# UCLA-VAST/soda-compiler

Hardware: AMD Instinct MI355X
Metric: gcell_updates_per_s (higher is better)
Workload: dtype f32; 1 GPU; jacobi2d.soda float32 16384x16384, iterate 1000; app=jacobi2d, valid_cell_updates=236970022000, nominal_cell_updates=268435456000, depth_schedule=41x24+1x16, depth_split=measured (soda_hip_plan_tune), stream_chunk_choice=calibrated (confirmed by measurement), device=gfx950:sramecc+:xnack-

## Files before the change

### soda-compiler_amd/csrc/schedule.cpp

```cpp
#include "schedule.h"

#include <algorithm>
#include <cmath>
#include <cstdarg>
#include <cstdio>
#include <cstdlib>
#include <cstring>

thread_local std::string g_last_error;

int fail(int code, const char* fmt, ...) {
  char buf[1024];
  va_list ap;
  va_start(ap, fmt);
  vsnprintf(buf, sizeof buf, fmt, ap);
  va_end(ap);
  g_last_error = buf;
  return code;
}

const char* tuning_env(const char* name) {
  const char* on = getenv("SODA_HIP_TUNING");
  return (on && on[0] == '1') ? getenv(name) : nullptr;
}
// ... 416 lines not shown
  if (desc.xcd_tiles && dim == 3) return place_super_tiles(plan, k, out);
  return 0;
}

int check_box_inside(const Planner* plan, const soda_hip_args& a,
                     const int32_t* reach_lo, const int32_t* reach_hi,
                     bool signed_window = false) {
  for (int d = 0; d < plan->prog.dim; ++d) {
    if (a.box_hi[d] <= a.box_lo[d]) continue;
    const int64_t first = signed_window ? a.box_lo[d] + reach_lo[d] : a.box_lo[d] - reach_lo[d];
    if (first < 0 || a.box_hi[d] + reach_hi[d] > a.dims[d])
      return fail(SODA_HIP_ERR_OUT_OF_BOUNDS,
                  "launch would read [%lld, %lld) of dimension %d, extent %lld",
                  (long long)first,
                  (long long)(a.box_hi[d] + reach_hi[d]), d, (long long)a.dims[d]);
  }
  return 0;
}

std::vector<int> eligible_fused(const Planner* plan, const int64_t* dims) {
  const soda_hip_program& p = plan->prog;
  std::vector<int> fused;
  for (size_t k = 0; k < plan->kernels.size(); ++k) {
    const soda_hip_kernel& kd = plan->kernels[k];
    if (kd.kind != SODA_HIP_KERNEL_FUSED ||
        (plan->max_depth > 0 && kd.depth > plan->max_depth))
      continue;
    if (kd.min_extent[0] > 0 &&
        (dims[0] < kd.min_extent[0] || (p.dim > 1 && dims[1] < kd.min_extent[1]) ||
         (p.dim > 2 && dims[0] * dims[1] >= (int64_t(1) << 30) - 16)))
      continue;
    fused.push_back((int)k);
  }
  std::sort(fused.begin(), fused.end(), [&](int a, int b) {
    return plan->kernels[a].depth > plan->kernels[b].depth;
  });
  return fused;
}

bool plans_fused(const Planner* plan, const std::vector<int>& fused, const int64_t* dims,
                 int iterate) {
  if (fused.empty() || plan->kernels[fused.back()].depth != 1) return false;
  if (plan->max_depth < 0) return false;
  if (plan->max_depth == 0 && !plan->tuning &&
      (takes_output_extras(plan, plan->kernels[fused.back()]) || plan->prog.dim == 1)) {
    return plan->tuned_split.find(split_key(plan, dims, iterate)) != plan->tuned_split.end();
  }
  return true;
}

soda_hip_args box_of_level(Planner* plan, Growth* g, const int64_t* dims, const int32_t* vlo,
                           const int32_t* vhi, int level, int32_t* mlo, int32_t* mhi) {
  const soda_hip_program& p = plan->prog;
  soda_hip_args a;
  memset(&a, 0, sizeof a);
  hull_margins(plan, g, level, mlo, mhi);
  for (int d = 0; d < SODA_HIP_MAX_DIMS; ++d) {
    a.dims[d] = d < p.dim ? dims[d] : 1;
    a.box_lo[d] = d < p.dim ? vlo[d] + mlo[d] : 0;
    a.box_hi[d] = d < p.dim ? dims[d] - vhi[d] - mhi[d] : 1;
  }
  return a;
}

int split_iterate(Planner* plan, Growth* g, const std::vector<int>& fused, const int64_t* dims,
                  int iterate, const int32_t* vlo, const int32_t* vhi, std::vector<int>* seq) {
  std::vector<int> usable;
// ... 104 lines not shown
                "carry the boxes of %d", desc.name, p.n_outputs, max_extra_outputs(dim));
  const std::vector<Box>& boxes = g->boxes[level - 1];
  for (int j = 0; j < p.n_outputs; ++j) {
    const Box& o = boxes[p.output_tensor[j]];
    int64_t ex[6];
    soda_hip_args own = *a;
    for (int d = 0; d < dim; ++d) {
      ex[d] = mlo[d] + o.lo[d];
      ex[dim + d] = mhi[d] - o.hi[d];
      if (ex[d] < 0 || ex[d] > kMaxExtra || ex[dim + d] < 0 || ex[dim + d] > kMaxExtra)
        return fail(SODA_HIP_ERR_INTERNAL, "kernel %s: output %d is %lld / %lld cells "
                    "wider than the launch's box in dimension %d (limit %d)", desc.name,
                    j, (long long)ex[d], (long long)ex[dim + d], d, kMaxExtra);
      own.box_lo[d] -= ex[d];
      own.box_hi[d] += ex[dim + d];
    }
    const int32_t none[SODA_HIP_MAX_DIMS] = {0, 0, 0, 0};
    int rc = check_box_inside(plan, own, none, none);
    if (rc) return rc;
    uint64_t word = 0;
    for (int i = 0; i < 2 * dim; ++i) word |= (uint64_t)ex[i] << (8 * i);
    if (dim == 1) a->param[1 + j / 4] |= (int64_t)(word << (16 * (j % 4)));
    else if (dim == 2) a->param[1 + j / 2] |= (int64_t)(word << (32 * (j % 2)));
    else a->param[1 + j] = (int64_t)word;
  }
  return 0;
}

int fused_list(Planner* plan, Growth* g, const std::vector<int>& fused, const std::vector<int>& seq,
               const int64_t* dims, const int32_t* vlo, const int32_t* vhi,
               std::vector<Launch>* list, int* max_depth_used, ScratchNeeds* needs) {
  const int m = (int)seq.size();
  int done = 0;
  std::vector<Buffer> src = sweep_inputs(plan);
  for (int i = 0; i < m; ++i) {
    const soda_hip_kernel& desc = plan->kernels[seq[i]];
    Buffer tensor[SODA_HIP_MAX_TENSORS];
    route(plan, i, m, &src, tensor, needs);
    int32_t mlo[SODA_HIP_MAX_DIMS], mhi[SODA_HIP_MAX_DIMS];
    int32_t plo[SODA_HIP_MAX_DIMS], phi[SODA_HIP_MAX_DIMS];
    hull_margins(plan, g, done, plo, phi);
    soda_hip_args a = box_of_level(plan, g, dims, vlo, vhi, done + desc.depth, mlo, mhi);
    int32_t reach_lo[SODA_HIP_MAX_DIMS], reach_hi[SODA_HIP_MAX_DIMS];
    for (int d = 0; d < SODA_HIP_MAX_DIMS; ++d) {
      reach_lo[d] = mlo[d] - plo[d];
      reach_hi[d] = mhi[d] - phi[d];
    }
    int rc = check_box_inside(plan, a, reach_lo, reach_hi);
    if (rc) return rc;
    if (takes_output_extras(plan, desc)) {
      rc = pack_output_extras(plan, g, desc, done + desc.depth, mlo, mhi, &a);
      if (rc) return rc;
    }
    Launch l;
    bool empty;
    rc = make_launch(plan, seq[i], a, &l, &empty);
    if (rc) return rc;
    if (!empty && l.est_us > 0) {
      const char* prefer = tuning_env("SODA_HIP_PREFER");
      auto preferred = [&](int k) {
        if (!prefer) return false;
        const size_t n = strlen(plan->kernels[k].name), m = strlen(prefer);
        return n >= m && strcmp(plan->kernels[k].name + n - m, prefer) == 0;
      };
      for (int k : fused) {
        if (k == seq[i] || plan->kernels[k].depth != desc.depth) continue;
        Launch other;
        bool other_empty;
        if (make_launch(plan, k, a, &other, &other_empty) == 0 && !other_empty &&
            other.est_us > 0 &&
            (preferred(k) || (other.est_us < l.est_us && !preferred(l.kernel))))
          l = other;
      }
    }
    std::copy(tensor, tensor + SODA_HIP_MAX_TENSORS, l.buffer);
    if (!empty) list->push_back(l);
    *max_depth_used = std::max(*max_depth_used, (int)desc.depth);
    done += desc.depth;
  }
  return 0;
}

int staged_list(Planner* plan, const Growth* g, const int64_t* dims, int iterate, const int32_t* vlo,
                const int32_t* vhi, std::vector<Launch>* list, int* max_depth_used,
                ScratchNeeds* needs) {
  const soda_hip_program& p = plan->prog;
  std::vector<int> stage_kernel(p.n_stages, -1);
  for (size_t k = 0; k < plan->kernels.size(); ++k)
    if (plan->kernels[k].kind == SODA_HIP_KERNEL_STAGE) {
      const int s = plan->kernels[k].stage - p.n_inputs;
      if (s >= 0 && s < p.n_stages) stage_kernel[s] = (int)k;
    }
  for (int s = 0; s < p.n_stages; ++s)
    if (stage_kernel[s] < 0)
      return fail(SODA_HIP_ERR_NO_KERNEL, "blob has no kernel for stage %d", s);
  std::vector<Buffer> src = sweep_inputs(plan);
  for (int it = 0; it < iterate; ++it) {
    Buffer tensor[SODA_HIP_MAX_TENSORS];
    for (int s = 0; s < p.n_stages; ++s) {
      if (is_output_tensor(p, p.n_inputs + s)) continue;
      tensor[p.n_inputs + s].kind = Buffer::LOCAL;
      tensor[p.n_inputs + s].index = (uint8_t)s;
      needs->locals = true;
    }
    route(plan, it, iterate, &src, tensor, needs);
// ... 95 lines not shown
```

### soda-compiler_amd/csrc/schedule.h

```cpp
#ifndef SODA_HIP_SCHEDULE_H_
#define SODA_HIP_SCHEDULE_H_

#include "soda_hip.h"

#include <array>
#include <cstdint>
#include <map>
#include <string>
#include <utility>
#include <vector>

struct Box {
  int32_t lo[SODA_HIP_MAX_DIMS];
  int32_t hi[SODA_HIP_MAX_DIMS];
  bool set;
};

struct Buffer {
  enum Kind : uint8_t {
    NONE,
    INPUT,
    OUTPUT,
    ARRAY_A,
    ARRAY_B,
// ... 16 lines not shown

struct ScratchNeeds {
  bool pingpong = false;
  bool second = false;
  bool locals = false;
};

struct Growth {
  std::vector<Box> start;
  std::vector<std::vector<Box>> boxes;
  std::vector<Box> feed;
};

struct Planner {
  soda_hip_program prog{};
  std::vector<soda_hip_kernel> kernels;
  std::vector<int> resident_blocks;
  std::vector<int> static_lds;
  int cus = 256;
  int64_t lds_per_cu = 160 * 1024;
  int max_depth = 0;
  int chunk_rows_override = 0;
  int chunk_rows_min = 8;
  int wgs_per_cu_cap = 0;
  bool out_final_only = false;
  int bias_depth = 0;
  double bias = 1.0;
  bool tuning = false;
  Growth fresh;
  std::map<std::vector<int32_t>, Growth> resumed;
  mutable std::map<std::array<int64_t, 4>, std::pair<int, int>> xcd_shape;
  std::map<std::array<int64_t, 5>, std::vector<int>> tuned_split;
  std::map<std::array<int64_t, 5>, std::array<int, 2>> tuned_stream;
};

#pragma GCC visibility push(hidden)

extern thread_local std::string g_last_error;
int fail(int code, const char* fmt, ...) __attribute__((format(printf, 2, 3)));

const char* tuning_env(const char* name);

int n_tensors(const soda_hip_program& p);
bool is_output_tensor(const soda_hip_program& p, int t);

void output_margins(Planner* plan, int iterations, int32_t* lo, int32_t* hi);
void field_margins(Planner* plan, int iterations, int32_t (*lo)[SODA_HIP_MAX_DIMS],
                   int32_t (*hi)[SODA_HIP_MAX_DIMS]);

std::array<int64_t, 5> split_key(const Planner* plan, const int64_t* dims, int iterate);
std::array<int64_t, 5> stream_key(const Planner* plan, int k, const soda_hip_args& args);

double footprint_of(const Planner* plan, const soda_hip_args& args);
const double kBeyondCacheBytes = 288.0 * 1024 * 1024;

int build_schedule(Planner* plan, const int64_t* dims, int iterate, const int32_t* valid_lo,
                   const int32_t* valid_hi, std::vector<Launch>* list, int* max_depth_used,
                   ScratchNeeds* needs);
int build_schedule_fields(Planner* plan, const int64_t* dims, int iterate,
                          const int32_t (*valid_lo)[SODA_HIP_MAX_DIMS],
                          const int32_t (*valid_hi)[SODA_HIP_MAX_DIMS],
                          std::vector<Launch>* list, int* max_depth_used, ScratchNeeds* needs);

#pragma GCC visibility pop

#endif
// ... 1 lines not shown
```

### soda-compiler_amd/csrc/soda_hip.cpp

```cpp
#include "plan.h"

#include <hip/hiprtc.h>

#include <algorithm>
#include <array>
#include <cmath>
#include <cstdio>
#include <cstdlib>
#include <cstring>
#include <map>
#include <string>
#include <vector>

namespace {

int grow_zeroed(void** array, size_t* have, size_t bytes, hipStream_t stream) {
  if (*have >= bytes) return 0;
  if (*array) {
    HIP_TRY(SODA_HIP_ERR_DEVICE_FREE, hipFree(*array));
    *array = nullptr;
    *have = 0;
  }
  HIP_TRY(SODA_HIP_ERR_DEVICE_MALLOC, hipMalloc(array, bytes));
  HIP_TRY(SODA_HIP_ERR_DEVICE_RUN, hipMemsetAsync(*array, 0, bytes, stream));
// ... 495 lines not shown
    int depth = 0;
    ScratchNeeds needs;
    rc = build_schedule(plan, dims, iterate, valid_lo, valid_hi, &list, &depth, &needs);
    std::vector<int> split;
    for (const Launch& l : list)
      if (plan->kernels[l.kernel].kind == SODA_HIP_KERNEL_FUSED)
        split.push_back(plan->kernels[l.kernel].depth);
    int total = 0;
    for (int d : split) total += d;
    if (!rc && total == iterate &&
        std::find(candidates.begin(), candidates.end(), split) == candidates.end())
      candidates.push_back(split);
  }
  plan->bias_depth = 0;
  plan->bias = 1.0;
  plan->tuning = false;
  if (rc) return rc;
  hipEvent_t e0 = nullptr, e1 = nullptr;
  if (hipEventCreate(&e0) != hipSuccess || hipEventCreate(&e1) != hipSuccess)
    return fail(SODA_HIP_ERR_DEVICE_RUN, "hipEventCreate failed");
  auto time_sweep = [&](int runs, float* fastest) -> int {
    int e = 0;
    for (int run = 0; run <= runs && !e; ++run) {
      if (hipEventRecord(e0, s) != hipSuccess) e = fail(SODA_HIP_ERR_DEVICE_RUN, "hipEventRecord failed");
      if (!e) e = soda_hip_sweep(plan, in, out, dims, iterate, valid_lo, valid_hi, stream);
      if (!e && (hipEventRecord(e1, s) != hipSuccess || hipEventSynchronize(e1) != hipSuccess))
        e = fail(SODA_HIP_ERR_DEVICE_SYNC, "timing a tuning sweep failed");
      float ms = 0;
      if (!e) (void)hipEventElapsedTime(&ms, e0, e1);
      if (run == 1 || (run > 1 && ms < *fastest)) *fastest = ms;
    }
    return e;
  };
  if (candidates.size() < 2) {
    rc = tune_streaming(plan, dims, iterate, valid_lo, valid_hi, time_sweep);
    (void)hipEventDestroy(e0);
    (void)hipEventDestroy(e1);
    return rc;
  }
  size_t best = 0;
  float best_ms = 0;
  for (size_t c = 0; c < candidates.size() && !rc; ++c) {
    plan->tuned_split[key] = candidates[c];
    float fastest = 0;
    rc = time_sweep(2, &fastest);
    if (tuning_env("SODA_HIP_DEBUG")) {
      fprintf(stderr, "soda_hip: tune %d iteration(s):", iterate);
      for (int d : candidates[c]) fprintf(stderr, " %d", d);
      fprintf(stderr, "  -> %.1f us\n", fastest * 1000.0);
    }
    if (c == 0 || fastest < best_ms) { best = c; best_ms = fastest; }
  }
  if (rc) plan->tuned_split.erase(key);
  else plan->tuned_split[key] = candidates[best];
  if (!rc) rc = tune_streaming(plan, dims, iterate, valid_lo, valid_hi, time_sweep);
  (void)hipEventDestroy(e0);
  (void)hipEventDestroy(e1);
  return rc;
}

int soda_hip_plan_set_split(soda_hip_plan* plan, const int64_t dims[SODA_HIP_MAX_DIMS],
                            int iterate, const int32_t* depths, int n_depths) {
  if (!plan || !dims) return fail(SODA_HIP_ERR_NULL_ARGUMENT, "NULL argument");
  const std::array<int64_t, 5> key = split_key(plan, dims, iterate);
  if (!depths || n_depths <= 0) {
    plan->tuned_split.erase(key);
    return 0;
  }
  int total = 0;
  for (int i = 0; i < n_depths; ++i) {
    bool known = false;
    for (const soda_hip_kernel& kd : plan->kernels)
      known = known || (kd.kind == SODA_HIP_KERNEL_FUSED && kd.depth == depths[i]);
    if (!known)
      return fail(SODA_HIP_ERR_NO_KERNEL, "no fused kernel of depth %d in the blob",
                  (int)depths[i]);
    total += depths[i];
  }
  if (total != iterate)
    return fail(SODA_HIP_ERR_CONSTRAINT, "the depths add up to %d, not to iterate = %d",
                total, iterate);
  plan->tuned_split[key] = std::vector<int>(depths, depths + n_depths);
  return 0;
}

int soda_hip_plan_set_out_final_only(soda_hip_plan* plan, int on) {
  if (!plan) return fail(SODA_HIP_ERR_NULL_ARGUMENT, "plan is NULL");
// ... 398 lines not shown
```

### soda-compiler_amd/soda_hip/codegen/kernel.py

```python
import collections
import functools
import hashlib
import inspect
import json
import os
import re
import subprocess
import tempfile

from .. import __version__
from . import (kernel_common, kernel_fields1d, kernel_fields2d, kernel_fields3d, kernel_stage,
               kernel_stream1d, kernel_stream2d, kernel_stream2d_wp, kernel_stream3d,
               kernel_stream3d_blk, kernel_stream3d_lds, kernel_stream3d_wp)
from . import spec as specmod
from . import switches

DEFAULT_MAX_DEPTH = 12
WAVE_GROUPS = -1
AUTO_WP_VGPRS = 200
AUTO_WP_GROUPS = 4
AUTO_WP_BUDGET = 200
AUTO_WP_RING = 6
AUTO_WP_SQUEEZE_VGPRS = 152
PACKED_DEEP_DEPTHS = (16, 20, 24)
PACKED_DEEP_DEPTH = PACKED_DEEP_DEPTHS[0]
PACKED_DEEP_WAVES_PER_EU = 3
PACKED_FROM_DEPTH = 12
WAVE_PIPELINE_MIN_DEPTH = 4
ALIGN_FULL_MAX_DEPTH = 2
NT_AUTO_MAX_DEPTH_2D = 2
EXACT_PREFETCH = 6
DEEP_3D_DEPTHS = (4,)
BLOCK_3D_SHALLOW_DEPTHS = (1, 2)
DEEP_3D_FORM = 'both'
BLOCK_3D_OPTIONS = dict(stack=8, prefetch=1, vgpr_budget=300, nt=4, mask_loads=1,
                        wide_stores=2, edge=1)
BLOCK_3D_RING_OPTIONS = dict(stack=8, prefetch=0, ring=2, vgpr_budget=300, nt=4,
                             mask_loads=1, wide_stores=2, lean_fill=1, edge=1)
DEEP_3D_MAX_WEIGHT = 20
PACKED_3D_LIGHT_WEIGHT = 10
ALIGN_FULL_MAX_WEIGHT = 40

FIELDS_DEPTHS = (1, 2, 4, 8)
FIELDS_OPTIONS = ('skip_fill', 'vgpr_budget', 'max_period', 'waves_per_eu')
FIELDS3D_DEPTHS = (1, 2)
FIELDS3D_OPTIONS = ('rows', 'vgpr_budget', 'max_period', 'waves_per_eu')
RECT3D_INPUT_ROWS = 36
STREAM1D_DEPTHS = (1, 2, 4, 8, 12)
STREAM1D_OPTIONS = ('segs',)
FIELDS1D_OPTIONS = STREAM1D_OPTIONS
LDS3D_OPTIONS = ('lds_shape',)

FAR_MAX_PERIOD = 24

SHARED_2D_OPTIONS = ('skip_fill', 'vgpr_budget', 'max_period', 'align', 'waves_per_eu')
WP_ONLY_OPTIONS = ('pairs', 'ring', 'split', 'prio', 'seam_probe')

HIPCC_FLAGS = ['-x', 'hip', '--offload-arch=gfx950', '--cuda-device-only',
               '--no-gpu-bundle-output', '-O3', '-ffp-contract=off',
               '-fno-slp-vectorize', '-fwrapv', '-std=c++17']


_DOUBLE_LITERAL = re.compile(
    r'(?<![\w.])(?:\d+\.\d*|\.\d+|\d+(?=[eE]))(?:[eE][+-]?\d+)?(?![\w.])')


def dpp_combine_is_safe(spec):
  if any(t != 'float' for t in specmod.tensor_c_types(spec).values()):
    return False
  for stage in spec['stages']:
    for text in [stage['expr']] + [l['expr'] for l in stage['lets']]:
      plain = specmod.LOAD_RE.sub('x', text)
      if _DOUBLE_LITERAL.search(plain) or kernel_common.used_functions(
          dict(stages=[dict(expr=text, lets=[])])) or 'static_cast<' in plain:
        return False
  return True


def extra_flags(spec):
  tuning = []
  if spec['dim'] == 2 and \
      kernel_stream2d_wp.packable(specmod.inline_pointwise(spec)):
    tuning = ['-mllvm', '-amdgpu-sched-strategy=max-ilp']
  if dpp_combine_is_safe(spec):
    return tuning
  return ['-mllvm', '-amdgpu-dpp-combine=false'] + tuning


FLAGS_MARK = '// SODA-HIP-FLAGS:'
# ... 116 lines not shown
    valu = waves * entry['depth'] * weight * lane_cells * 2
    cells_in = waves * kernel_stream2d.LANES * lane_cells
    cells_out = entry['tile'][0] * entry['tile'][1]
  entry['step_valu'] = int(valu)
  entry['step_bytes'] = int((n_in * cells_in + n_out * cells_out) * elem)
  measured = calibration().get(calibration_key(entry, spec))
  if measured:
    for field in CALIBRATED_FIELDS:
      entry[field] = int(measured.get(field, 0))
    for field in MEASURED_OVER_DEFAULT:
      if field in measured:
        entry[field] = int(measured[field])
  return entry


def prefixed_options(options, prefix, emit):
  known = inspect.signature(emit).parameters
  out = {}
  for key, value in options.items():
    if key.startswith(prefix):
      if key[len(prefix):] not in known:
        raise TypeError('%s: %s() has no option `%s`' % (key, emit.__module__,
                                                         key[len(prefix):]))
      out[key[len(prefix):]] = value
  return out



FORM_OPTIONS = dict(
    fields2d=lambda k: k in FIELDS_OPTIONS,
    fields3d=lambda k: k in FIELDS3D_OPTIONS,
    fields1d=lambda k: k in FIELDS1D_OPTIONS,
    stream1d=lambda k: k in STREAM1D_OPTIONS,
    stream2d=lambda k: k not in WP_ONLY_OPTIONS + STREAM1D_OPTIONS and k != 'nt',
    stream2d_wp=lambda k: k in SHARED_2D_OPTIONS + WP_ONLY_OPTIONS,
    stream3d=lambda k: not k.startswith(('wp_', 'blk_')) and
    k not in ('deep3d', 'deep3d_from', 'nontemporal') + STREAM1D_OPTIONS + LDS3D_OPTIONS,
    stream3d_lds=lambda k: k in LDS3D_OPTIONS)
PREFIXED_FORMS = dict(stream3d_blk=('blk_', kernel_stream3d_blk.emit),
                      stream3d_wp=('wp_', kernel_stream3d_wp.emit))


def form_options(form, options):
  if form in PREFIXED_FORMS:
    return prefixed_options(options, *PREFIXED_FORMS[form])
  return {k: v for k, v in options.items() if FORM_OPTIONS[form](k)}


def first_fusable(spec, depth, attempts):
  error = None
  for emit, kwargs in attempts:
    try:
      return emit(spec, depth, **kwargs), None
    except kernel_stream2d.NotFusable as e:
      error = e
  return None, error


class Request:

  def __init__(self, spec, max_depth, cols, chunk_rows, prefetch, depths, wave_groups,
               options, on):
    self.spec, self.depths, self.options = spec, depths, options
    self.on = {s.keyword: bool(on[s.keyword]) for s in switches.SWITCHES}
    self.meta_notes, self.made = {}, []
    self.far = {}
    fuse_outputs = self.on['fuse_outputs']
    self.rect = fuse_outputs and kernel_stream2d.rectangular(spec)
    if fuse_outputs and not self.rect and len(spec['outputs']) >= 2 and \
        spec['dim'] in (2, 3) and not kernel_stream2d.multi_field(spec):
# ... 199 lines not shown


def stream2d_piped(req, depth, strip, notes):
  spec, groups = req.spec, req.groups
  options = form_options('stream2d_wp', req.options)
  if groups == -1:
    options.setdefault('vgpr_budget', AUTO_WP_BUDGET)
    lane_bytes = strip['cols'] * specmod.ELEM_SIZE[spec['inputs'][0]['c_type']]
    if lane_bytes == 16:
      options.setdefault('ring', AUTO_WP_RING)
    options.setdefault('pairs', 0 if not kernel_stream2d_wp.packable(spec)
                       else 2 if options.get('ring') else 1)
    if depth > PACKED_DEEP_DEPTH and options['pairs'] == 2:
      options.setdefault('waves_per_eu', PACKED_DEEP_WAVES_PER_EU)
  emit = kernel_stream2d_wp.emit
  piped, error = first_fusable(spec, depth, [
      (emit, dict(strip, groups=AUTO_WP_GROUPS if groups == -1 else groups, **options))])
  if piped is not None and squeeze(req, options, piped[1]):
    capped = None
    if options.get('pairs') == 2 and options['ring'] == AUTO_WP_RING \
        and 'max_period' not in options:
      capped = dict(options, ring=2 * AUTO_WP_RING, max_period=2 * AUTO_WP_RING)
    elif not options.get('pairs'):
      capped = options
    if capped is not None:
      again, error = first_fusable(spec, depth, [
          (emit, dict(strip, groups=AUTO_WP_GROUPS, waves_per_eu=4, **capped))])
      piped = again or piped
  if error is not None:
    notes.append('depth %d not wave-pipelined: %s' % (depth, error))
  return piped


def stream2d_kernels(req, notes):
  spec = req.spec
  if spec['dim'] != 2 or kernel_stream2d.multi_field(spec) or req.rect:
    return
  far = req.far
  for depth in stream2d_depths(req):
    strip = dict(req.strip)
    if 'align' not in req.options:
      strip['align'] = 'full' if (
          depth <= ALIGN_FULL_MAX_DEPTH and
          arithmetic_weight(spec) <= ALIGN_FULL_MAX_WEIGHT) else 'none'
    single = piped = None
    if req.groups <= 1 or depth < WAVE_PIPELINE_MIN_DEPTH:
      single = stream2d_single(req, depth, strip, notes, far)
    if want_piped(req, depth, single):
      piped = stream2d_piped(req, depth, strip, notes)
      if piped is None and single is None and req.groups > 1:
        single, error = first_fusable(spec, depth, [
            (kernel_stream2d.emit,
             dict(strip, **dict(far, **form_options('stream2d', req.options))))])
        if single is None:
          notes.append('depth %d not fused: %s' % (depth, error))
    if piped is not None or single is not None:
      yield piped if piped is not None else single


def stream3d_kernels(req, notes):
  spec, cols = req.spec, req.cols
  if spec['dim'] != 3 or kernel_stream2d.multi_field(spec) or req.rect:
    return
  wanted = req.default_depths
  if req.depths is not None:
    wanted = sorted(set([1] + list(req.depths))) if req.chain else [1]
  for depth in wanted:
    options = form_options('stream3d', req.options)
    narrow = [] if cols or len(spec['inputs']) == len(spec['outputs']) else \
        [(12, 1), (16, 1)]
    shapes = [(options.pop('rows'), cols or 2)] if 'rows' in options else \
        [(16, cols or 2), (12, cols or 2)] + narrow
    options.setdefault('nt', 4)
    found, error = first_fusable(spec, depth, [
        (kernel_stream3d.emit, dict(options, rows=rows, cols=lane_cols))
        for rows, lane_cols in shapes])
    if found is None:
      notes.append('depth %d not fused: %s' % (depth, error))
    else:
      yield found


def deep3d_block(req, depth, notes):
  spec = req.spec
  given = form_options('stream3d_blk', req.options)
  heavy = arithmetic_weight(spec) > PACKED_3D_LIGHT_WEIGHT
  ring_forms = [dict(BLOCK_3D_RING_OPTIONS)]
  if heavy and kernel_stream2d_wp.packable(spec):
    ring_forms.insert(0, dict(BLOCK_3D_RING_OPTIONS, pairs=1, wide_stores=0))
# ... 147 lines not shown
```

### soda-compiler_amd/soda_hip/codegen/kernel_stream2d_wp.py

```python
import re

from . import spec as specmod
from .kernel_common import builtin_type, cell_assignment, device_expr, tensor_index
from .kernel_stream2d import LANES, Instance, NotFusable, geometry, kernel_name


def build_groups(spec, depth, prefetch, groups, loader=False, split=None, sync=1,
                 ring_lag=1):
  axis = spec['dim'] - 1
  if len(spec['outputs']) != 1 or len(spec['inputs']) != 1:
    raise NotFusable('one input, one output')
  types = specmod.tensor_c_types(spec)
  if len({specmod.ELEM_SIZE[t] for t in types.values()}) != 1:
    raise NotFusable('mixed element widths')
  in_name = spec['inputs'][0]['name']
  source = Instance('in_%s' % in_name, in_name, 0, types[in_name])
  source.role, source.group = 'global_in', 0
  stages = []
  current = {in_name: source}
  for it in range(depth):
    for stage in spec['stages']:
      inst = Instance('k%d_%s' % (it, stage['name']), stage['name'], it,
                      stage['c_type'], stage)
      inst.role = 'compute'
# ... 57 lines not shown
    inst.lag = lag
  everything = [source] + stages + list(copies.values()) + ([ring] if loader else [])
  for inst in stages:
    for src, rel, _ in inst.reads:
      src.keep = max(src.keep, inst.lag - rel[axis] - src.lag + 1)
  for inst in stages:
    if inst.role == 'compute' and not inst.final and inst.keep == 0:
      raise NotFusable('stage %s is never read' % inst.tensor)
  per_wave = []
  for g in range(groups):
    mine = [ring if loader else source] if g == 0 else [copies[id(last_of[g - 1])]]
    mine += stages[bounds[g]:bounds[g + 1]]
    per_wave.append(mine)
  return everything, per_wave, final


PLAIN_FLOAT_EXPR = re.compile(
    r'^(?:\{[^}]*\}|(?:\d+\.?\d*|\.\d+)(?:[eE][+-]?\d+)?f|\d+|[-+*/() ])*$')


def packable(spec):
  if any(t != 'float' for t in specmod.tensor_c_types(spec).values()):
    return False
  for stage in spec['stages']:
    if stage['lets']:
      return False
    if not PLAIN_FLOAT_EXPR.match(device_expr(stage['expr'])):
      return False
  return True


def emit(spec, depth, cols=None, chunk_rows=256, prefetch=3, groups=4,
         max_period=12, vgpr_budget=120, skip_fill=1, pairs=0, align='none',
         ring=0, waves_per_eu=0, split=None, prio=None, seam_probe=0):
  types = specmod.tensor_c_types(spec)
  index = tensor_index(spec)
  in_type = spec['inputs'][0]['c_type']
  out_name = spec['outputs'][0]
  elem = specmod.ELEM_SIZE[in_type]
  if cols is None:
    cols = max(1, 16 // elem)
  C = cols
  if pairs and not packable(spec):
    raise NotFusable('packed form: float programs of + - * / only')
  if pairs and (C * elem) % 16:
    raise NotFusable('packed form: whole 16-byte vectors per lane')
  P = 2 if pairs else 1
  wide = int(pairs) == 2
  if spec['dim'] != 2:
    raise NotFusable('2-D programs only')
  RS = int(ring)
  PF = RS - 2
  if RS and (RS < 3 or C * elem != 16):
    raise NotFusable('input ring: >= 3 slots, 16-byte lanes')
  if wide and not RS:
    raise NotFusable('wide strips come through the input ring')
  if isinstance(split, str):
    split = [int(v) for v in split.split('/')]
  everything, per_wave, final = build_groups(spec, depth, 0 if RS else prefetch,
                                             groups, split=split)
  S = 1
  dppadd = int(pairs) == 1
  geo = geometry(spec, depth, C, chunk_rows, align)
  if wide:
    geo['w_out'] += LANES * C
  strip_cols = LANES * C * (2 if wide else 1)
  for inst in everything:
    for src, rel, _ in inst.reads:
      if abs(rel[0]) > C:
        raise NotFusable('x offset %d exceeds the %d columns a lane holds'
                         % (rel[0], C))
  best = None
  for candidate in range(2, max_period + 1, 2):
    if max(i.keep for i in everything) > candidate:
      continue
    if RS and candidate % RS:
      continue
    if candidate % (2 * S):
      continue
    divisors = [d for d in range(1, candidate + 1) if candidate % d == 0]
    padded = [min(d for d in divisors if d >= i.keep) if i.keep else 0
              for i in everything]
    cost = (sum(padded), candidate)
    if best is None or cost < best[0]:
      best = (cost, candidate, padded)
  if best is None:
    raise NotFusable('windows exceed the rotation period limit')
  period = best[1]
  for inst, keep in zip(everything, best[2]):
    inst.keep = keep
  per_elem = max(1, elem // 4)
  est_vgprs = max(sum(i.keep for i in mine) for mine in per_wave) * C * per_elem * P + \
      4 * C * P + 20
  if est_vgprs > vgpr_budget:
    raise NotFusable('a wavefront would need about %d VGPRs (budget %d)'
                     % (est_vgprs, vgpr_budget))
  below = {id(final): 0}
  order = [i for mine in per_wave for i in mine]
  for inst in reversed(order):
    need = below.get(id(inst))
    if need is None:
      continue
    if inst.role == 'lds_in':
      below[id(inst.origin)] = max(below.get(id(inst.origin), -10**9), need)
    for src, rel, _ in inst.reads:
      below[id(src)] = max(below.get(id(src), -10**9), need - rel[1])
  for inst in everything:
    inst.first_step = max(0, inst.lag + geo['y_lo'] - below.get(id(inst), 0))
  name = kernel_name(spec, depth)
  L = final.lag
  T_in = builtin_type(in_type)
  T_out = builtin_type(types[out_name])
  vec = 'vec_%s' % name
  o = []
  line = o.append
  line('// fused depth-%d kernel, wave-pipelined: %d wavefronts per strip, rotation '
       'period %d,' % (depth, groups, period))
  line('// strip = %d columns (%d out + halo %d/%d), prefetch %d rows, ~%d VGPRs'
       % (strip_cols, geo['w_out'], geo['halo_lo'], geo['halo_hi'], prefetch,
          est_vgprs))
  for g, mine in enumerate(per_wave):
    for inst in mine:
      line('//   wave %d  %-20s lag %2d keep %2d  %s' % (
          g, inst.ident, inst.lag, inst.keep,
          '-> HBM' if inst.final else inst.role))
  line('typedef %s %s __attribute__((ext_vector_type(%d), aligned(%d)));'
       % (T_in, vec, C, elem))
  line('typedef %s %s_lds __attribute__((ext_vector_type(%d), aligned(%d)));'
       % (T_in, vec, C, C * elem))
  if pairs:
    line('typedef float pk2 __attribute__((ext_vector_type(2)));')
  pieces = C * P * elem // 16 if pairs else 1
  per_piece = C * P // pieces

  def slot(inst, u, back):
    return (u - back) % inst.keep

  def operand(reader, src, rel, u, c):
    back = reader.lag - src.lag - rel[1]
    assert 0 <= back < src.keep, (reader.ident, src.ident, rel, back, src.keep)
    row = '%s[%d]' % (src.ident, slot(src, u, back))
    j = c + rel[0]
    if 0 <= j < C:
      return '%s[%d]' % (row, j)
    if wide:
      return 'pk_wide_%s(%s[%d])' % (('below', row, C + j) if j < 0 else
                                     ('above', row, j - C))
    shift = 'pk_from_lane' if pairs and dppadd else 'from_lane'
    if j < 0:
      return '%s_below(%s[%d])' % (shift, row, C + j)
    return '%s_above(%s[%d])' % (shift, row, j - C)

  def vmcnt(n):
    return (n & 15) | (7 << 4) | (15 << 8) | ((n >> 4) << 14)

  def ring_issue(row_expr, slot_index):
    line('        { i64 row = %s; if (row > H - 1) row = H - 1;' % row_expr)
    for h in range(P):
      line('          __builtin_amdgcn_global_load_lds((const __attribute__(('
           'address_space(1))) void*)(g_in + row * W + %s), (__attribute__(('
           'address_space(3))) void*)&in_ring[%d][%d][0], 16, 0, %d);'
           % (('x - lane * %d + %d' % (C, h * LANES * C)) if wide else
              ('xb' if h else 'x'), slot_index, h, 0))
    line('        }')

  def emit_body(mine, guarded):
    probed = [i for i in mine if i.role in ('compute', 'lds_out') or i.final] if seam_probe \
        else []
    for u in range(period):
      line('      {  // unrolled step %d' % u)
      for inst in mine:
        if inst.role == 'global_in' and RS:
          s = slot(inst, u, 0)
          ring_issue('head + %d' % (u + PF), (u + PF) % RS)
          line('        __builtin_amdgcn_s_waitcnt(%d);  // vmcnt(%d)'
               % (vmcnt(PF * P), PF * P))
          if wide and C == 4:
            line('        soda_lds_read_pairs4(&in_ring[%d][0][0] + lane * 8, %s);'
                 % (u % RS, ', '.join('%s[%d][%d]' % (inst.ident, s, c)
                                      for c in range(C))))
            continue
          for h in range(P):
            line('        const %s_lds ring_v%d = __builtin_bit_cast(%s_lds, '
                 'soda_lds_read_f4(&in_ring[%d][%d][0] + lane * %d + %d));'
                 % (vec, h, vec, u % RS, 0 if wide else h, C * (2 if wide else 1),
                    C * h if wide else 0))
          for c in range(C):
            line('        %s[%d][%d] = %s;' % (
                inst.ident, s, c,
                'pk2{ring_v0[%d], ring_v1[%d]}' % (c, c) if pairs else 'ring_v0[%d]' % c))
          continue
        if inst.role == 'global_in':
          s = slot(inst, u, 0)
          line('        { i64 row = head + %d; if (row > H - 1) row = H - 1;' % u)
          line('          const %s* p = g_in + row * W + x;' % T_in)
          if pairs:
            line('          if (INTERIOR) { const %s va = *(const %s*)p, vb = *(const %s*)'
                 '(p + %d);%s }' % (vec, vec, vec, geo['w_out'], ''.join(
                     ' %s[%d][%d] = pk2{va[%d], vb[%d]};' % (inst.ident, s, c, c, c)
                     for c in range(C))))
            line('          else {%s } }' % ''.join(
                ' %s[%d][%d] = pk2{(x + %d >= 0 && x + %d < W) ? p[%d] : 0.0f, '
                '(x + %d >= 0 && x + %d < W) ? p[%d] : 0.0f};'
                % (inst.ident, s, c, c, c, c, c + geo['w_out'], c + geo['w_out'],
                   c + geo['w_out']) for c in range(C)))
            continue
          line('          if (INTERIOR) { const %s v = *(const %s*)p;%s }' % (
              vec, vec, ''.join(' %s[%d][%d] = v[%d];' % (inst.ident, s, c, c)
                                for c in range(C))))
# ... 24 lines not shown
        direct = inst.keep == 0
        if direct:
          line('        %s out_row[%d];' % (ctype, C))
        for c in range(C):
          def load(tensor, rel, u=u, c=c, inst=inst, by_name=by_name):
            return operand(inst, by_name[(tensor, tuple(rel))], tuple(rel), u, c)
          target = ('out_row[%d]' % c) if direct else \
              '%s[%d][%d]' % (inst.ident, slot(inst, u, 0), c)
          cell_assignment(stage, target, load, line, '        ')
        if inst in probed:
          k = probed.index(inst)
          row = 'out_row' if direct else '%s[%d]' % (inst.ident, slot(inst, u, 0))
          line('        { float seam_in;')
          line('          asm volatile("ds_read_b32 %%0, %%1 offset:%d\\n\\ts_waitcnt lgkmcnt(0)" '
               ': "=v"(seam_in) : "v"(seam_rd + %du));' % (k * 256, ((u + 1) % 2) * 2048))
          line('          seam_acc += seam_in; }')
          line('        { const float e = seam_first ? %s[0][0] : %s[%d][1];' % (row, row, C - 1))
          line('          asm volatile("ds_write_b32 %%0, %%1 offset:%d" :: "v"(seam_wr + %du), '
               '"v"(e)); }' % (k * 256, (u % 2) * 2048))
        if inst.role == 'lds_out' and pairs:
          for q in range(pieces):
            line('        { soda_f4 v;%s *(soda_f4*)&handoff[%d][%d][%d][%d][lane * 4] = v; }' % (
                ''.join(' v[%d] = out_row[%d][0]; v[%d] = out_row[%d][1];' % (
                    2 * j, q * 2 + j, 2 * j + 1, q * 2 + j) for j in range(2)),
                inst.handoff, (u // S) % 2, u % S, q))
        elif inst.role == 'lds_out':
          line('        { %s_lds v;%s *(%s_lds*)&handoff[%d][%d][%d][lane * %d] = v; }' % (
              vec, ''.join(' v[%d] = out_row[%d];' % (c, c) for c in range(C)),
              vec, inst.handoff, (u // S) % 2, u % S, C))
        if inst.final:
          line('        { const i64 y = head + %d;' % (u - L))
          line('          if (y >= y0 && y < y1) {')
          line('            if (!ragged) {')
          for half in range(P):
            sel = '[%d]' % half if pairs else ''
            xv = 'xb' if half else 'x'
            line('              if (full_%d) { %s v;%s *(%s*)(g_out + y * W + %s) = v; }'
                 % (half, vec, ''.join(' v[%d] = out_row[%d]%s;' % (c, c, sel)
                                       for c in range(C)), vec, xv))
          line('            } else {')
          for half in range(P):
            sel = '[%d]' % half if pairs else ''
            sfx = 'b' if half and not wide else ''
            xv = 'xb' if half else 'x'
            line('            { %s* q = g_out + y * W + %s;' % (T_out, xv))
            line('            if (%s >= st_lo%s && %s + %d <= st_hi%s) { %s v;%s '
                 '*(%s*)q = v; }'
                 % (xv, sfx, xv, C, sfx, vec, ''.join(
                     ' v[%d] = out_row[%d]%s;' % (c, c, sel) for c in range(C)), vec))
            line('            else {%s } }' % ''.join(
                ' if (%s + %d >= st_lo%s && %s + %d < st_hi%s) q[%d] = out_row[%d]%s;'
                % (xv, c, sfx, xv, c, sfx, c, c, sel) for c in range(C)))
          line('            }')
          line('          } }')
        if skip:
          line('        }')
      line('      }')
      if (u + 1) % S == 0:
        line('      %s();' % ('soda_lds_barrier' if RS else 'soda_block_barrier'))

  line('template <bool INTERIOR>')
  line('DEV void %s_strip(const soda_hip_args& a, const i64 xs, const i64 x, '
       'const i64 xb, const i64 y0, const i64 y1, const int wave, const int lane,'
       % name)
  ring_dims = (P, LANES * C) if RS else (1, 1)
  if pairs and seam_probe:
    line('    float (*handoff)[2][%d][%d][%d], %s (*in_ring)[%d][%d], float* seam_lds) {'
         % (S, pieces, LANES * 4, T_in, ring_dims[0], ring_dims[1]))
  elif pairs:
    line('    float (*handoff)[2][%d][%d][%d], %s (*in_ring)[%d][%d]) {'
         % (S, pieces, LANES * 4, T_in, ring_dims[0], ring_dims[1]))
  else:
    line('    %s (*handoff)[2][%d][%d], %s (*in_ring)[%d][%d]) {'
         % (T_in, S, LANES * C, T_in, ring_dims[0], ring_dims[1]))
  line('  const i64 W = a.dims[0], H = a.dims[1];')
  line('  const i64 st_lo = xs > a.box_lo[0] ? xs : a.box_lo[0];')
  line('  const i64 st_hi = xs + %d < a.box_hi[0] ? xs + %d : a.box_hi[0];'
       % (geo['w_out'], geo['w_out']))
  if pairs and not wide:
    line('  const i64 st_lob = xs + %d;' % geo['w_out'])
    line('  const i64 st_hib = xs + %d < a.box_hi[0] ? xs + %d : a.box_hi[0];'
         % (2 * geo['w_out'], 2 * geo['w_out']))
    line('  (void)st_lob; (void)st_hib;')
  line('  const %s* __restrict__ g_in = (const %s*)a.tensor[%d];'
       % (T_in, T_in, index[spec['inputs'][0]['name']]))
  line('  %s* __restrict__ g_out = (%s*)a.tensor[%d];' % (T_out, T_out,
                                                           index[out_name]))
  line('  (void)g_in; (void)g_out; (void)st_lo; (void)st_hi; (void)W; (void)H; '
       '(void)xb; (void)in_ring;')
  parts = []
  for half in range(P):
    sfx = 'b' if half and pairs and not wide else ''
    xv = 'xb' if half else 'x'
    line('  const bool full_%d = %s >= st_lo%s && %s + %d <= st_hi%s; (void)full_%d;'
         % (half, xv, sfx, xv, C, sfx, half))
    parts.append('(!full_%d && %s + %d > st_lo%s && %s < st_hi%s)'
                 % (half, xv, C, sfx, xv, sfx))
  line('  const bool ragged = __builtin_amdgcn_ballot_w64(%s) != 0; (void)ragged;'
       % ' || '.join(parts))
  line('  const i64 steps = (y1 - y0) + %d;' % (L + geo['y_lo']))
  if seam_probe:
    line('  float seam_acc = 0.0f;')
    line('  const bool seam_first = lane == 0;')
    line('  const unsigned seam_wr = (unsigned)(unsigned long long)seam_lds + wave * 4096u + '
         'lane * 4u;')
    line('  const unsigned seam_rd = (unsigned)(unsigned long long)seam_lds + wave * 4096u + '
         '(63 - lane) * 4u;')
  prologue_steps = max(i.first_step for i in everything)
  prologue_steps = -(-prologue_steps // period) * period if skip_fill else 0
  for g, mine in enumerate(per_wave):
    line('  %sif (wave == %d) {' % ('' if g == 0 else 'else ', g))
    levels = [3] + [0] * (groups - 1) if prio is None else \
        ([int(v) for v in (prio if isinstance(prio, (list, tuple)) else str(prio).split('/'))] + [0] * groups)[:groups]
    if levels[g]:
      line('    __builtin_amdgcn_s_setprio(%d);' % levels[g])
    for inst in mine:
      if inst.keep:
        line('    %s %s[%d][%d];' % ('pk2' if pairs else builtin_type(inst.c_type),
                                     inst.ident, inst.keep, C))
        for r in range(inst.keep):
          line('    ' + ' '.join('%s[%d][%d] = %s;' % (
              inst.ident, r, c, 'pk2{0.0f, 0.0f}' if pairs else '0')
                                 for c in range(C)))
    line('    i64 head = y0 - %d;' % geo['y_lo'])
# ... 82 lines not shown
```

Before: 8364 Gcell-updates/s.

## Add 12-column packed wavefront kernel variant for deep depths with tuned form selection

Adds a new fused 2-D kernel form for depths 20 and 24, using 6 columns per lane with packed pairs (12 columns per lane). Input arrives through the LDS ring via multiple 16-byte global_load_lds pieces and is read back with inline ds_read_b32. The planner gains a per-problem 'form' choice, timed during tuning, that forces the first or last same-depth candidate. Candidate selection also prefers kernels with measured step costs. The aim is more reuse per lane and better choice between variants, at the cost of higher VGPR pressure (2 waves per EU) and more tuning time.

```diff
diff --git a/soda-compiler_amd/csrc/schedule.cpp b/soda-compiler_amd/csrc/schedule.cpp
--- a/soda-compiler_amd/csrc/schedule.cpp
+++ b/soda-compiler_amd/csrc/schedule.cpp
@@ -472,7 +472,7 @@
       continue;
     fused.push_back((int)k);
   }
-  std::sort(fused.begin(), fused.end(), [&](int a, int b) {
+  std::stable_sort(fused.begin(), fused.end(), [&](int a, int b) {
     return plan->kernels[a].depth > plan->kernels[b].depth;
   });
   return fused;
@@ -643,6 +643,10 @@
                std::vector<Launch>* list, int* max_depth_used, ScratchNeeds* needs) {
   const int m = (int)seq.size();
   int done = 0;
+  int iterate = 0, form = 0;
+  for (int k : seq) iterate += plan->kernels[k].depth;
+  const auto tuned_form = plan->tuned_form.find(split_key(plan, dims, iterate));
+  if (tuned_form != plan->tuned_form.end()) form = tuned_form->second;
   std::vector<Buffer> src = sweep_inputs(plan);
   for (int i = 0; i < m; ++i) {
     const soda_hip_kernel& desc = plan->kernels[seq[i]];
@@ -674,14 +678,30 @@
         const size_t n = strlen(plan->kernels[k].name), m = strlen(prefer);
         return n >= m && strcmp(plan->kernels[k].name + n - m, prefer) == 0;
       };
+      auto measured = [&](int k) {
+        return plan->kernels[k].step_ns_full > 0 && plan->kernels[k].step_ns_one > 0;
+      };
+      int first = -1, last = -1;
+      for (int k : fused)
+        if (plan->kernels[k].depth == desc.depth) {
+          if (first < 0) first = k;
+          last = k;
+        }
+      const int forced = form == 1 ? first : form == 2 ? last : -1;
       for (int k : fused) {
         if (k == seq[i] || plan->kernels[k].depth != desc.depth) continue;
         Launch other;
         bool other_empty;
-        if (make_launch(plan, k, a, &other, &other_empty) == 0 && !other_empty &&
-            other.est_us > 0 &&
-            (preferred(k) || (other.est_us < l.est_us && !preferred(l.kernel))))
-          l = other;
+        if (make_launch(plan, k, a, &other, &other_empty) != 0 || other_empty ||
+            other.est_us <= 0)
+          continue;
+        if (forced >= 0 && !prefer) {
+          if (k == forced) l = other;
+          continue;
+        }
+        const bool cheaper = measured(k) != measured(l.kernel) ? measured(k)
+                                                               : other.est_us < l.est_us;
+        if (preferred(k) || (cheaper && !preferred(l.kernel))) l = other;
       }
     }
     std::copy(tensor, tensor + SODA_HIP_MAX_TENSORS, l.buffer);
diff --git a/soda-compiler_amd/csrc/schedule.h b/soda-compiler_amd/csrc/schedule.h
--- a/soda-compiler_amd/csrc/schedule.h
+++ b/soda-compiler_amd/csrc/schedule.h
@@ -72,6 +72,7 @@
   mutable std::map<std::array<int64_t, 4>, std::pair<int, int>> xcd_shape;
   std::map<std::array<int64_t, 5>, std::vector<int>> tuned_split;
   std::map<std::array<int64_t, 5>, std::array<int, 2>> tuned_stream;
+  std::map<std::array<int64_t, 5>, int> tuned_form;
 };
 
 #pragma GCC visibility push(hidden)
diff --git a/soda-compiler_amd/csrc/soda_hip.cpp b/soda-compiler_amd/csrc/soda_hip.cpp
--- a/soda-compiler_amd/csrc/soda_hip.cpp
+++ b/soda-compiler_amd/csrc/soda_hip.cpp
@@ -551,8 +551,38 @@
     }
     return e;
   };
+  auto tune_forms = [&]() -> int {
+    std::vector<Launch> list;
+    int depth = 0;
+    ScratchNeeds needs;
+    int e = build_schedule(plan, dims, iterate, valid_lo, valid_hi, &list, &depth, &needs);
+    bool several = false;
+    for (const Launch& l : list) {
+      const soda_hip_kernel& kd = plan->kernels[l.kernel];
+      if (kd.kind != SODA_HIP_KERNEL_FUSED) continue;
+      for (size_t k = 0; k < plan->kernels.size(); ++k)
+        several = several || ((int)k != l.kernel && plan->kernels[k].depth == kd.depth &&
+                              plan->kernels[k].kind == SODA_HIP_KERNEL_FUSED);
+    }
+    if (e || !several) return e;
+    int best_form = 0;
+    float best_form_ms = 0;
+    for (int form = 0; form < 3 && !e; ++form) {
+      plan->tuned_form[key] = form;
+      float fastest = 0;
+      e = time_sweep(2, &fastest);
+      if (tuning_env("SODA_HIP_DEBUG"))
+        fprintf(stderr, "soda_hip: tune %d iteration(s): form %d -> %.1f us\n", iterate, form,
+                fastest * 1000.0);
+      if (form == 0 || fastest < best_form_ms) { best_form = form; best_form_ms = fastest; }
+    }
+    if (e) plan->tuned_form.erase(key);
+    else plan->tuned_form[key] = best_form;
+    return e;
+  };
   if (candidates.size() < 2) {
-    rc = tune_streaming(plan, dims, iterate, valid_lo, valid_hi, time_sweep);
+    rc = tune_forms();
+    if (!rc) rc = tune_streaming(plan, dims, iterate, valid_lo, valid_hi, time_sweep);
     (void)hipEventDestroy(e0);
     (void)hipEventDestroy(e1);
     return rc;
@@ -572,6 +602,7 @@
   }
   if (rc) plan->tuned_split.erase(key);
   else plan->tuned_split[key] = candidates[best];
+  if (!rc) rc = tune_forms();
   if (!rc) rc = tune_streaming(plan, dims, iterate, valid_lo, valid_hi, time_sweep);
   (void)hipEventDestroy(e0);
   (void)hipEventDestroy(e1);
diff --git a/soda-compiler_amd/soda_hip/codegen/kernel.py b/soda-compiler_amd/soda_hip/codegen/kernel.py
--- a/soda-compiler_amd/soda_hip/codegen/kernel.py
+++ b/soda-compiler_amd/soda_hip/codegen/kernel.py
@@ -25,6 +25,10 @@
 PACKED_DEEP_DEPTHS = (16, 20, 24)
 PACKED_DEEP_DEPTH = PACKED_DEEP_DEPTHS[0]
 PACKED_DEEP_WAVES_PER_EU = 3
+WIDE12_DEPTHS = (20, 24)
+WIDE12_OPTIONS = dict(cols=6, pairs=2, ring=AUTO_WP_RING, waves_per_eu=2, vgpr_budget=256,
+                      suffix='w')
+WIDE12_DEFAULT = 1
 PACKED_FROM_DEPTH = 12
 WAVE_PIPELINE_MIN_DEPTH = 4
 ALIGN_FULL_MAX_DEPTH = 2
@@ -55,6 +59,7 @@
 
 SHARED_2D_OPTIONS = ('skip_fill', 'vgpr_budget', 'max_period', 'align', 'waves_per_eu')
 WP_ONLY_OPTIONS = ('pairs', 'ring', 'split', 'prio', 'seam_probe')
+SELECT_2D_OPTIONS = ('wide12',)
 
 HIPCC_FLAGS = ['-x', 'hip', '--offload-arch=gfx950', '--cuda-device-only',
                '--no-gpu-bundle-output', '-O3', '-ffp-contract=off',
@@ -237,10 +242,12 @@
     fields3d=lambda k: k in FIELDS3D_OPTIONS,
     fields1d=lambda k: k in FIELDS1D_OPTIONS,
     stream1d=lambda k: k in STREAM1D_OPTIONS,
-    stream2d=lambda k: k not in WP_ONLY_OPTIONS + STREAM1D_OPTIONS and k != 'nt',
+    stream2d=lambda k: k not in WP_ONLY_OPTIONS + STREAM1D_OPTIONS + SELECT_2D_OPTIONS and
+    k != 'nt',
     stream2d_wp=lambda k: k in SHARED_2D_OPTIONS + WP_ONLY_OPTIONS,
     stream3d=lambda k: not k.startswith(('wp_', 'blk_')) and
-    k not in ('deep3d', 'deep3d_from', 'nontemporal') + STREAM1D_OPTIONS + LDS3D_OPTIONS,
+    k not in ('deep3d', 'deep3d_from', 'nontemporal') + STREAM1D_OPTIONS + LDS3D_OPTIONS +
+    SELECT_2D_OPTIONS,
     stream3d_lds=lambda k: k in LDS3D_OPTIONS)
 PREFIXED_FORMS = dict(stream3d_blk=('blk_', kernel_stream3d_blk.emit),
                       stream3d_wp=('wp_', kernel_stream3d_wp.emit))
@@ -506,6 +513,20 @@
   return piped
 
 
+def stream2d_wide12(req, depth, strip, piped, notes):
+  how = int(req.options.get('wide12', WIDE12_DEFAULT))
+  if not how or depth not in WIDE12_DEPTHS or req.groups != -1 or req.cols or \
+      piped is None or piped[1].get('pairs') != 2 or piped[1]['cols'] != 4:
+    return None
+  options = dict(WIDE12_OPTIONS, **{k: v for k, v in form_options('stream2d_wp', req.options).items()
+                                    if k not in WIDE12_OPTIONS})
+  found, error = first_fusable(req.spec, depth, [
+      (kernel_stream2d_wp.emit, dict(dict(strip, groups=AUTO_WP_GROUPS), **options))])
+  if found is None:
+    notes.append('depth %d not in 12-column lanes: %s' % (depth, error))
+  return found
+
+
 def stream2d_kernels(req, notes):
   spec = req.spec
   if spec['dim'] != 2 or kernel_stream2d.multi_field(spec) or req.rect:
@@ -528,7 +549,11 @@
              dict(strip, **dict(far, **form_options('stream2d', req.options))))])
         if single is None:
           notes.append('depth %d not fused: %s' % (depth, error))
-    if piped is not None or single is not None:
+    wide12 = stream2d_wide12(req, depth, strip, piped, notes)
+    if wide12 is not None:
+      yield wide12
+    if (piped is not None or single is not None) and not (
+        wide12 is not None and int(req.options.get('wide12', WIDE12_DEFAULT)) == 2):
       yield piped if piped is not None else single
 
 
diff --git a/soda-compiler_amd/soda_hip/codegen/kernel_stream2d_wp.py b/soda-compiler_amd/soda_hip/codegen/kernel_stream2d_wp.py
--- a/soda-compiler_amd/soda_hip/codegen/kernel_stream2d_wp.py
+++ b/soda-compiler_amd/soda_hip/codegen/kernel_stream2d_wp.py
@@ -113,7 +113,7 @@
 
 def emit(spec, depth, cols=None, chunk_rows=256, prefetch=3, groups=4,
          max_period=12, vgpr_budget=120, skip_fill=1, pairs=0, align='none',
-         ring=0, waves_per_eu=0, split=None, prio=None, seam_probe=0):
+         ring=0, waves_per_eu=0, split=None, prio=None, seam_probe=0, suffix=''):
   types = specmod.tensor_c_types(spec)
   index = tensor_index(spec)
   in_type = spec['inputs'][0]['c_type']
@@ -124,16 +124,19 @@
   C = cols
   if pairs and not packable(spec):
     raise NotFusable('packed form: float programs of + - * / only')
-  if pairs and (C * elem) % 16:
-    raise NotFusable('packed form: whole 16-byte vectors per lane')
   P = 2 if pairs else 1
   wide = int(pairs) == 2
+  wide12 = wide and C * elem == 24
+  if pairs and (C * elem) % 16 and not wide12:
+    raise NotFusable('packed form: whole 16-byte vectors per lane')
   if spec['dim'] != 2:
     raise NotFusable('2-D programs only')
   RS = int(ring)
   PF = RS - 2
-  if RS and (RS < 3 or C * elem != 16):
+  if RS and (RS < 3 or (C * elem != 16 and not wide12)):
     raise NotFusable('input ring: >= 3 slots, 16-byte lanes')
+  if wide12 and (not RS or seam_probe):
+    raise NotFusable('12-column lanes: through the input ring, no seam probe')
   if wide and not RS:
     raise NotFusable('wide strips come through the input ring')
   if isinstance(split, str):
@@ -146,6 +149,9 @@
   if wide:
     geo['w_out'] += LANES * C
   strip_cols = LANES * C * (2 if wide else 1)
+  if wide12:
+    geo['origin_align'] = 4
+  NQ = 2 * C * elem // 16 if wide12 else P
   for inst in everything:
     for src, rel, _ in inst.reads:
       if abs(rel[0]) > C:
@@ -173,6 +179,8 @@
   per_elem = max(1, elem // 4)
   est_vgprs = max(sum(i.keep for i in mine) for mine in per_wave) * C * per_elem * P + \
       4 * C * P + 20
+  if wide12:
+    est_vgprs = max(sum(i.keep for i in mine) for mine in per_wave) * C * P + C * P + 12 + 16
   if est_vgprs > vgpr_budget:
     raise NotFusable('a wavefront would need about %d VGPRs (budget %d)'
                      % (est_vgprs, vgpr_budget))
@@ -188,7 +196,7 @@
       below[id(src)] = max(below.get(id(src), -10**9), need - rel[1])
   for inst in everything:
     inst.first_step = max(0, inst.lag + geo['y_lo'] - below.get(id(inst), 0))
-  name = kernel_name(spec, depth)
+  name = kernel_name(spec, depth) + suffix
   L = final.lag
   T_in = builtin_type(in_type)
   T_out = builtin_type(types[out_name])
@@ -206,9 +214,10 @@
           g, inst.ident, inst.lag, inst.keep,
           '-> HBM' if inst.final else inst.role))
   line('typedef %s %s __attribute__((ext_vector_type(%d), aligned(%d)));'
-       % (T_in, vec, C, elem))
-  line('typedef %s %s_lds __attribute__((ext_vector_type(%d), aligned(%d)));'
-       % (T_in, vec, C, C * elem))
+       % (T_in, vec, 4 if wide12 else C, elem))
+  if not wide12:
+    line('typedef %s %s_lds __attribute__((ext_vector_type(%d), aligned(%d)));'
+         % (T_in, vec, C, C * elem))
   if pairs:
     line('typedef float pk2 __attribute__((ext_vector_type(2)));')
   pieces = C * P * elem // 16 if pairs else 1
@@ -237,7 +246,12 @@
 
   def ring_issue(row_expr, slot_index):
     line('        { i64 row = %s; if (row > H - 1) row = H - 1;' % row_expr)
-    for h in range(P):
+    for q in range(NQ if wide12 else 0):
+      line('          __builtin_amdgcn_global_load_lds((const __attribute__(('
+           'address_space(1))) void*)(g_in + row * W + x), (__attribute__(('
+           'address_space(3))) void*)(&in_ring[%d][%d][0] - %d), 16, %d, 0);'
+           % (slot_index, q, 4 * q, 16 * q))
+    for h in range(0 if wide12 else P):
       line('          __builtin_amdgcn_global_load_lds((const __attribute__(('
            'address_space(1))) void*)(g_in + row * W + %s), (__attribute__(('
            'address_space(3))) void*)&in_ring[%d][%d][0], 16, 0, %d);'
@@ -245,8 +259,17 @@
               ('xb' if h else 'x'), slot_index, h, 0))
     line('        }')
 
+  piece_x = ['x'] + ['xq%d' % q for q in range(1, NQ)]
+
+  def piece_value(q, j):
+    k = 4 * q + j
+    return 'out_row[%d][%d]' % (k % C, k // C)
+
+  def piece_values(q):
+    return ''.join(' v[%d] = %s;' % (j, piece_value(q, j)) for j in range(4))
+
   def emit_body(mine, guarded):
-    probed = [i for i in mine if i.role in ('compute', 'lds_out') or i.final] if seam_probe \
+    probed =[i for i in mine if i.role in ('compute', 'lds_out') or i.final] if seam_probe \
         else []
     for u in range(period):
       line('      {  // unrolled step %d' % u)
@@ -255,7 +278,21 @@
           s = slot(inst, u, 0)
           ring_issue('head + %d' % (u + PF), (u + PF) % RS)
           line('        __builtin_amdgcn_s_waitcnt(%d);  // vmcnt(%d)'
-               % (vmcnt(PF * P), PF * P))
+               % (vmcnt(PF * NQ), PF * NQ))
+          if wide12:
+            row_bytes = NQ * LANES * 16
+            names = ['f%d' % k for k in range(2 * C)]
+            line('        { float %s;' % ', '.join(names))
+            line('          asm volatile("%s\\n\\ts_waitcnt lgkmcnt(0)" : %s : "v"(ring_rd) : '
+                 '"memory");' % (
+                     '\\n\\t'.join('ds_read_b32 %%%d, %%%d offset:%d' % (
+                         k, 2 * C, (u % RS) * row_bytes + (k // 4) * LANES * 16 + (k % 4) * 4)
+                                   for k in range(2 * C)),
+                     ', '.join('"=&v"(%s)' % n for n in names)))
+            for c in range(C):
+              line('          %s[%d][%d] = pk2{f%d, f%d};' % (inst.ident, s, c, c, c + C))
+            line('        }')
+            continue
           if wide and C == 4:
             line('        soda_lds_read_pairs4(&in_ring[%d][0][0] + lane * 8, %s);'
                  % (u % RS, ', '.join('%s[%d][%d]' % (inst.ident, s, c)
@@ -346,14 +383,25 @@
           line('        { const i64 y = head + %d;' % (u - L))
           line('          if (y >= y0 && y < y1) {')
           line('            if (!ragged) {')
-          for half in range(P):
+          for q in range(NQ if wide12 else 0):
+            line('              if (full_%d) { %s v;%s *(%s*)(g_out + y * W + %s) = v; }'
+                 % (q, vec, piece_values(q), vec, piece_x[q]))
+          for half in range(0 if wide12 else P):
             sel = '[%d]' % half if pairs else ''
             xv = 'xb' if half else 'x'
             line('              if (full_%d) { %s v;%s *(%s*)(g_out + y * W + %s) = v; }'
                  % (half, vec, ''.join(' v[%d] = out_row[%d]%s;' % (c, c, sel)
                                        for c in range(C)), vec, xv))
           line('            } else {')
-          for half in range(P):
+          for q in range(NQ if wide12 else 0):
+            xv = piece_x[q]
+            line('            { %s* q = g_out + y * W + %s;' % (T_out, xv))
+            line('            if (%s >= st_lo && %s + 4 <= st_hi) { %s v;%s *(%s*)q = v; }'
+                 % (xv, xv, vec, piece_values(q), vec))
+            line('            else {%s } }' % ''.join(
+                ' if (%s + %d >= st_lo && %s + %d < st_hi) q[%d] = %s;'
+                % (xv, j, xv, j, j, piece_value(q, j)) for j in range(4)))
+          for half in range(0 if wide12 else P):
             sel = '[%d]' % half if pairs else ''
             sfx = 'b' if half and not wide else ''
             xv = 'xb' if half else 'x'
@@ -377,7 +425,7 @@
   line('DEV void %s_strip(const soda_hip_args& a, const i64 xs, const i64 x, '
        'const i64 xb, const i64 y0, const i64 y1, const int wave, const int lane,'
        % name)
-  ring_dims = (P, LANES * C) if RS else (1, 1)
+  ring_dims = (NQ, LANES * 4) if wide12 else (P, LANES * C) if RS else (1, 1)
   if pairs and seam_probe:
     line('    float (*handoff)[2][%d][%d][%d], %s (*in_ring)[%d][%d], float* seam_lds) {'
          % (S, pieces, LANES * 4, T_in, ring_dims[0], ring_dims[1]))
@@ -403,7 +451,18 @@
   line('  (void)g_in; (void)g_out; (void)st_lo; (void)st_hi; (void)W; (void)H; '
        '(void)xb; (void)in_ring;')
   parts = []
-  for half in range(P):
+  if wide12:
+    line('  const i64 %s; %s' % (
+        ', '.join('xq%d = x + %d' % (q, 4 * q) for q in range(1, NQ)),
+        ' '.join('(void)xq%d;' % q for q in range(1, NQ))))
+    line('  const unsigned ring_rd = (unsigned)(unsigned long long)&in_ring[0][0][0] + '
+         'lane * 16u; (void)ring_rd;')
+    for q in range(NQ):
+      xv = piece_x[q]
+      line('  const bool full_%d = %s >= st_lo && %s + 4 <= st_hi; (void)full_%d;'
+           % (q, xv, xv, q))
+      parts.append('(!full_%d && %s + 4 > st_lo && %s < st_hi)' % (q, xv, xv))
+  for half in range(0 if wide12 else P):
     sfx = 'b' if half and pairs and not wide else ''
     xv = 'xb' if half else 'x'
     line('  const bool full_%d = %s >= st_lo%s && %s + %d <= st_hi%s; (void)full_%d;'
```

After: 8450 Gcell-updates/s (median of 6 runs). 1.01x the previous value.
